# LargeWorldModel/LWM

Hardware: NVIDIA H100
Metric: ring_attn_fwd_bwd_tokens_per_s_attention_only_7B_128K (higher is better)
Workload: dtype bf16

## Files before the change

lwm_b200/csrc/attn_fwd.cu:

```cuda
#include "attn_common.cuh"
#include "tmap.h"
#include "capi_internal.h"

namespace lwm {

struct FwdParams {
  int B, H, Sq, Sk;
  float scale_log2;
  MaskParams mask;
  __nv_bfloat16* out;
  float* out_f32;
  float* lse;
  float* acc_o;
  float* acc_m;
  float* acc_l;
  int first, last;
  const float *scale_q, *scale_k, *scale_v;
};

constexpr int kFwdStages = 4;
constexpr int kFwdTileBytes = kTile * kHeadDim * 2;
constexpr int kFwdThreads = 384;
constexpr int kFwdConsumerWarps = 8;
constexpr int kFwdSmemBytes = (1 + kFwdStages) * kFwdTileBytes + 1024;

struct FwdBarriers {
  uint64_t q_full;
  uint64_t kv_full[kFwdStages];
  uint64_t kv_empty[kFwdStages];
};

LWM_DEVICE void load_tile(uint8_t* dst, const CUtensorMap* tm, uint64_t* bar, int h, int row0, int b) {
  mbar_arrive_expect_tx(bar, kFwdTileBytes);
  tma_load_4d(dst, tm, bar, 0, h, row0, b);
  tma_load_4d(dst + kFwdTileBytes / 2, tm, bar, 64, h, row0, b);
}

LWM_DEVICE float quad_max(float x) {
  x = fmaxf(x, __shfl_xor_sync(0xffffffffu, x, 1));
  return fmaxf(x, __shfl_xor_sync(0xffffffffu, x, 2));
}
LWM_DEVICE float quad_sum(float x) {
  x += __shfl_xor_sync(0xffffffffu, x, 1);
  return x + __shfl_xor_sync(0xffffffffu, x, 2);
}

template <bool kF16>
__global__ void __launch_bounds__(kFwdThreads, 1)
attn_fwd_kernel(const __grid_constant__ CUtensorMap tmQ, const __grid_constant__ CUtensorMap tmK,
                const __grid_constant__ CUtensorMap tmV, const FwdParams p) {
  extern __shared__ uint8_t smem_raw[];
  uint8_t* smem = reinterpret_cast<uint8_t*>((reinterpret_cast<uintptr_t>(smem_raw) + 1023) & ~uintptr_t(1023));
  uint8_t* sQ = smem;
  uint8_t* sKV = smem + kFwdTileBytes;
  __shared__ FwdBarriers bars;

  const int warp = threadIdx.x >> 5;
  const int lane = threadIdx.x & 31;
  const int n_q_tiles = p.Sq / kTile;
  const int tile = n_q_tiles - 1 - int(blockIdx.x);
  const int h = blockIdx.y, b = blockIdx.z;
  const int m0 = tile * kTile;

  int n_kv = p.Sk / kTile;
  if (p.mask.causal) {
    const long long last_q = (long long)p.mask.q_pos0 + m0 + kTile - 1;
    const long long vis = last_q - p.mask.k_pos0;
    n_kv = vis < 0 ? 0 : min((long long)n_kv, vis / kTile + 1);
  }
  if (n_kv == 0 && !p.first && !p.last) return;

  if (threadIdx.x == 0) {
    mbar_init(&bars.q_full, 1);
    for (int i = 0; i < kFwdStages; ++i) {
      mbar_init(&bars.kv_full[i], 1);
      mbar_init(&bars.kv_empty[i], kFwdConsumerWarps);
    }
    fence_mbar_init();
  }
  __syncthreads();

  if (warp >= 8) {
    setmaxnreg_dec<40>();
    if (warp == 8 && lane == 0 && n_kv > 0) {
      tma_prefetch_desc(&tmQ);
      tma_prefetch_desc(&tmK);
      tma_prefetch_desc(&tmV);
      load_tile(sQ, &tmQ, &bars.q_full, h, m0, b);
      for (int i = 0; i < 2 * n_kv; ++i) {
        const int slot = i % kFwdStages;
        const uint32_t ph = (i / kFwdStages) & 1;
        mbar_wait(&bars.kv_empty[slot], ph ^ 1);
        load_tile(sKV + slot * kFwdTileBytes, (i & 1) ? &tmV : &tmK, &bars.kv_full[slot], h, (i >> 1) * kTile, b);
      }
    }
    return;
  }

  setmaxnreg_inc<232>();
  const int wg = warp >> 2;
  const int w = warp & 3;
  const int quad = lane & 3;
  const int r0 = m0 + wg * 64 + w * 16 + (lane >> 2);
  const float scale = p.scale_log2 * (p.scale_q ? (*p.scale_q) * (*p.scale_k) : 1.0f);
  const bool has_bias = p.mask.bias != nullptr, has_seg = p.mask.seg != nullptr;
  const float* bias_row = has_bias ? p.mask.bias + (long long)b * p.mask.bias_stride : nullptr;
  const int* seg_row = has_seg ? p.mask.seg + (long long)b * p.mask.seg_stride : nullptr;
  long long q_pos[2];
  int my_seg[2];
#pragma unroll
  for (int hh = 0; hh < 2; ++hh) {
    q_pos[hh] = (long long)p.mask.q_pos0 + r0 + 8 * hh;
    my_seg[hh] = has_seg ? seg_row[q_pos[hh]] : 0;
  }

  float o[64];
#pragma unroll
  for (int i = 0; i < 64; ++i) o[i] = 0.f;
  float m_run[2] = {-INFINITY, -INFINITY}, l_run[2] = {0.f, 0.f};

  if (n_kv > 0) {
    mbar_wait(&bars.q_full, 0);
    const uint64_t q_desc = desc_kmajor_sw128(smem_u32(sQ + wg * 64 * 128));
    const uint32_t kv_base = smem_u32(sKV);
    const long long warp_q_pos0 = (long long)p.mask.q_pos0 + m0 + wg * 64 + w * 16;
    for (int j = 0; j < n_kv; ++j) {
      const int ik = 2 * j, iv = 2 * j + 1;
      float s[64];
      mbar_wait(&bars.kv_full[ik % kFwdStages], (ik / kFwdStages) & 1);
      const uint64_t kd = desc_kmajor_sw128(kv_base + (ik % kFwdStages) * kFwdTileBytes);
      wgmma_fence();
#pragma unroll
      for (int ks = 0; ks < kHeadDim / 16; ++ks) {
        const uint32_t off = (ks >> 2) * (kFwdTileBytes / 2) + (ks & 3) * 32;
        wgmma_ss<128, kF16, 0, 0>(s, desc_advance(q_desc, off), desc_advance(kd, off), ks > 0);
      }
      wgmma_commit();
      wgmma_wait<0>();
      reg_fence(s);
      if (lane == 0) mbar_arrive(&bars.kv_empty[ik % kFwdStages]);

      const long long k_tile_pos = (long long)p.mask.k_pos0 + (long long)j * kTile;
      const bool need_mask = has_bias || has_seg || (p.mask.causal && (k_tile_pos + kTile - 1 > warp_q_pos0));
      float mx[2] = {-INFINITY, -INFINITY};
      if (!need_mask) {
#pragma unroll
        for (int i = 0; i < 64; ++i) mx[(i >> 1) & 1] = fmaxf(mx[(i >> 1) & 1], s[i]);
        mx[0] = quad_max(mx[0]) * scale;
        mx[1] = quad_max(mx[1]) * scale;
      } else {
#pragma unroll
        for (int i = 0; i < 64; ++i) {
          const int hh = (i >> 1) & 1;
          const int col = (i >> 2) * 8 + quad * 2 + (i & 1);
          float tv = s[i] * scale;
          if (has_bias) {
            const float bt = bias_row[k_tile_pos + col] * kLog2e;
            tv = (bt < kMaskedLogit) ? kMaskedLogit : tv + bt;
          }
          if (has_seg && seg_row[k_tile_pos + col] != my_seg[hh]) tv = kMaskedLogit;
          if (p.mask.causal && k_tile_pos + col > q_pos[hh]) tv = kMaskedLogit;
          s[i] = tv;
          mx[hh] = fmaxf(mx[hh], tv);
        }
        mx[0] = quad_max(mx[0]);
        mx[1] = quad_max(mx[1]);
      }
      float alpha[2];
#pragma unroll
      for (int hh = 0; hh < 2; ++hh) {
        const float m_new = fmaxf(m_run[hh], mx[hh]);
        alpha[hh] = (m_run[hh] == -INFINITY) ? 0.f : ex2f(m_run[hh] - m_new);
        m_run[hh] = m_new;
        l_run[hh] *= alpha[hh];
      }
      if (j > 0) {
#pragma unroll
        for (int i = 0; i < 64; ++i) o[i] *= alpha[(i >> 1) & 1];
      }
      const float neg_m[2] = {-m_run[0], -m_run[1]};
      uint32_t pa[8][4];
#pragma unroll
      for (int kk = 0; kk < 8; ++kk) {
        float e[8];
#pragma unroll
        for (int t = 0; t < 8; ++t) {
          const int i = 8 * kk + t;
          const int hh = (t >> 1) & 1;
          e[t] = need_mask ? ex2f(s[i] + neg_m[hh]) : ex2f(fmaf(s[i], scale, neg_m[hh]));
          l_run[hh] += e[t];
        }
#pragma unroll
        for (int t = 0; t < 4; ++t) pa[kk][t] = kF16 ? pack_f16x2(e[2 * t], e[2 * t + 1]) : pack_bf16x2(e[2 * t], e[2 * t + 1]);
      }

      mbar_wait(&bars.kv_full[iv % kFwdStages], (iv / kFwdStages) & 1);
      const uint64_t vd = desc_mnmajor_sw128(kv_base + (iv % kFwdStages) * kFwdTileBytes, kFwdTileBytes / 2);
      reg_fence(o);
      wgmma_fence();
#pragma unroll
      for (int kk = 0; kk < kTile / 16; ++kk) wgmma_rs128<kF16, 1>(o, pa[kk], desc_advance(vd, kk * 2048), 1);
      wgmma_commit();
      wgmma_wait<0>();
      reg_fence(o);
      if (lane == 0) mbar_arrive(&bars.kv_empty[iv % kFwdStages]);
    }
  }

#pragma unroll
  for (int hh = 0; hh < 2; ++hh) {
    const int q_row = r0 + 8 * hh;
    const float l_run_row = quad_sum(l_run[hh]);
    const long long ml_idx = ((long long)b * p.H + h) * p.Sq + q_row;
    const long long o_idx = (((long long)b * p.Sq + q_row) * p.H + h) * kHeadDim;
    float m_c = -INFINITY, l_c = 0.f;
    if (!p.first) {
      m_c = p.acc_m[ml_idx];
      l_c = p.acc_l[ml_idx];
    }
    const float m_new = fmaxf(m_c, m_run[hh]);
    float wa = (m_c == -INFINITY) ? 0.f : ex2f(m_c - m_new);
    float wb = (m_run[hh] == -INFINITY) ? 0.f : ex2f(m_run[hh] - m_new);
    const float l_new = wa * l_c + wb * l_run_row;
    if (p.scale_v) wb *= *p.scale_v;
    if (p.last) {
      const float inv = l_new > 0.f ? 1.0f / l_new : 0.f;
      wa *= inv;
      wb *= inv;
    }
#pragma unroll
    for (int g = 0; g < kHeadDim / 8; ++g) {
      const int c = g * 8 + quad * 2;
      float2 f = make_float2(o[4 * g + 2 * hh] * wb, o[4 * g + 2 * hh + 1] * wb);
      if (!p.first) {
        const float2 a2 = *reinterpret_cast<const float2*>(p.acc_o + o_idx + c);
        f.x = fmaf(a2.x, wa, f.x);
        f.y = fmaf(a2.y, wa, f.y);
      }
      if (p.last) {
        *reinterpret_cast<uint32_t*>(p.out + o_idx + c) = pack_bf16x2(f.x, f.y);
        if (p.out_f32) *reinterpret_cast<float2*>(p.out_f32 + o_idx + c) = f;
      } else {
        *reinterpret_cast<float2*>(p.acc_o + o_idx + c) = f;
      }
    }
    if (quad == 0) {
      if (p.last) {
        p.lse[ml_idx] = l_new > 0.f ? (m_new + log2f(l_new)) * kLn2 : -INFINITY;
      } else {
        p.acc_m[ml_idx] = m_new;
        p.acc_l[ml_idx] = l_new;
      }
    }
  }
}

static bool make_qkv_tmap(CUtensorMap* tm, const void* ptr, int B, int S, int H) {
  uint64_t dims[4] = {uint64_t(kHeadDim), uint64_t(H), uint64_t(S), uint64_t(B)};
  uint64_t strides[3] = {uint64_t(kHeadDim) * 2, uint64_t(H) * kHeadDim * 2, uint64_t(S) * H * kHeadDim * 2};
  uint32_t box[4] = {64, 1, uint32_t(kTile), 1};
  return encode_tmap(tm, CU_TENSOR_MAP_DATA_TYPE_BFLOAT16, 4, ptr, dims, strides, box, CU_TENSOR_MAP_SWIZZLE_128B);
}

}

using namespace lwm;

static int attn_fwd_launch(const void* q, const void* k, const void* v, void* out, float* lse, float* acc_o,
                           float* acc_m, float* acc_l, int B, int H, int Sq, int Sk, int D, long long q_pos0,
                           long long k_pos0, int causal, const float* bias, long long bias_stride,
                           const int* segment_ids, long long seg_stride, float softmax_scale, int first, int last,
                           const float* scale_q, const float* scale_k, const float* scale_v, float* out_f32,
                           void* stream) {
  if (D != kHeadDim) return lwm_fail(LWM_ERR_SHAPE, "attn_fwd: head_dim must be 128");
  if (B <= 0 || H <= 0 || Sq <= 0 || Sk <= 0 || Sq % kTile || Sk % kTile)
    return lwm_fail(LWM_ERR_SHAPE, "attn_fwd: Sq and Sk must be positive multiples of 128");
  if (!q || !k || !v) return lwm_fail(LWM_ERR_ARG, "attn_fwd: null q/k/v");
  if (last && (!out || !lse)) return lwm_fail(LWM_ERR_ARG, "attn_fwd: out/lse required on the last step");
  if (!(first && last) && (!acc_o || !acc_m || !acc_l))
    return lwm_fail(LWM_ERR_ARG, "attn_fwd: carry buffers required unless first && last");
  if (q_pos0 + Sq > 0x7fffffffLL || k_pos0 + Sk > 0x7fffffffLL)
    return lwm_fail(LWM_ERR_SHAPE, "attn_fwd: global positions must fit in int32");
  if (bias && bias_stride < k_pos0 + Sk)
    return lwm_fail(LWM_ERR_SHAPE, "attn_fwd: bias is indexed by GLOBAL key position: bias_stride < k_pos0 + Sk");
  if (segment_ids && (seg_stride < q_pos0 + Sq || seg_stride < k_pos0 + Sk))
    return lwm_fail(LWM_ERR_SHAPE, "attn_fwd: segment_ids is indexed by GLOBAL position: seg_stride < max(q_pos0 + Sq, k_pos0 + Sk)");
  if (!lwm_check_device()) return LWM_ERR_DEVICE;
  CUtensorMap tq, tk, tv;
  if (!make_qkv_tmap(&tq, q, B, Sq, H) || !make_qkv_tmap(&tk, k, B, Sk, H) || !make_qkv_tmap(&tv, v, B, Sk, H))
    return lwm_fail(LWM_ERR_CUDA, "attn_fwd: cuTensorMapEncodeTiled failed (pointers must be 16B aligned)");
  FwdParams p;
  p.B = B; p.H = H; p.Sq = Sq; p.Sk = Sk;
  p.scale_log2 = softmax_scale * kLog2e;
  p.mask.q_pos0 = int(q_pos0); p.mask.k_pos0 = int(k_pos0); p.mask.causal = causal;
  p.mask.bias = bias; p.mask.bias_stride = bias_stride;
  p.mask.seg = segment_ids; p.mask.seg_stride = seg_stride;
  p.out = reinterpret_cast<__nv_bfloat16*>(out);
  p.lse = lse; p.acc_o = acc_o; p.acc_m = acc_m; p.acc_l = acc_l;
  p.first = first; p.last = last;
  p.scale_q = scale_q; p.scale_k = scale_k; p.scale_v = scale_v;
  p.out_f32 = out_f32;
  static bool attr_set_dev[64] = {};
  int cur_dev = 0;
  cudaGetDevice(&cur_dev);
  bool& attr_set = attr_set_dev[cur_dev & 63];
  if (!attr_set) {
    if (cudaFuncSetAttribute(attn_fwd_kernel<false>, cudaFuncAttributeMaxDynamicSharedMemorySize, kFwdSmemBytes) !=
            cudaSuccess ||
        cudaFuncSetAttribute(attn_fwd_kernel<true>, cudaFuncAttributeMaxDynamicSharedMemorySize, kFwdSmemBytes) !=
            cudaSuccess)
      return lwm_fail(LWM_ERR_CUDA, "attn_fwd: cannot raise dynamic shared memory limit");
    attr_set = true;
  }
  dim3 grid(Sq / kTile, H, B);
  if (scale_q)
    attn_fwd_kernel<true><<<grid, kFwdThreads, kFwdSmemBytes, reinterpret_cast<cudaStream_t>(stream)>>>(tq, tk, tv, p);
  else
    attn_fwd_kernel<false><<<grid, kFwdThreads, kFwdSmemBytes, reinterpret_cast<cudaStream_t>(stream)>>>(tq, tk, tv, p);
  return lwm_check_launch("attn_fwd_kernel");
}

extern "C" int lwm_attn_fwd_step(const void* q, const void* k, const void* v, void* out, float* lse, float* acc_o,
                                 float* acc_m, float* acc_l, int B, int H, int Sq, int Sk, int D,
                                 long long q_pos0, long long k_pos0, int causal, const float* bias,
                                 long long bias_stride, const int* segment_ids, long long seg_stride,
                                 float softmax_scale, int first, int last, void* stream) {
  return attn_fwd_launch(q, k, v, out, lse, acc_o, acc_m, acc_l, B, H, Sq, Sk, D, q_pos0, k_pos0, causal, bias,
                         bias_stride, segment_ids, seg_stride, softmax_scale, first, last, nullptr, nullptr, nullptr, nullptr, stream);
}

extern "C" int lwm_attn_fwd_step_f16(const void* q16, const void* k16, const void* v16, const float* scale_q,
                                     const float* scale_k, const float* scale_v, float* out_f32,
                                     void* out, float* lse, float* acc_o, float* acc_m, float* acc_l, int B, int H,
                                     int Sq, int Sk, int D, long long q_pos0, long long k_pos0, int causal,
                                     const float* bias, long long bias_stride, const int* segment_ids,
                                     long long seg_stride, float softmax_scale, int first, int last, void* stream) {
  if (!scale_q || !scale_k || !scale_v) return lwm_fail(LWM_ERR_ARG, "attn_fwd_f16: scales required");
  return attn_fwd_launch(q16, k16, v16, out, lse, acc_o, acc_m, acc_l, B, H, Sq, Sk, D, q_pos0, k_pos0, causal, bias,
                         bias_stride, segment_ids, seg_stride, softmax_scale, first, last, scale_q, scale_k, scale_v,
                         out_f32, stream);
}
```

lwm_b200/csrc/ptx.cuh:

```cuda
#pragma once
#include <cuda.h>
#include <cuda_runtime.h>
#include <cuda_bf16.h>
#include <stdint.h>
#include "wgmma.cuh"

namespace lwm {

#define LWM_DEVICE __device__ __forceinline__

LWM_DEVICE uint32_t smem_u32(const void* p) {
  return static_cast<uint32_t>(__cvta_generic_to_shared(p));
}
LWM_DEVICE uint32_t lane_id() { return threadIdx.x & 31; }

LWM_DEVICE void mbar_init(uint64_t* bar, uint32_t count) {
  asm volatile("mbarrier.init.shared::cta.b64 [%0], %1;" ::"r"(smem_u32(bar)), "r"(count) : "memory");
}
LWM_DEVICE void fence_mbar_init() { asm volatile("fence.mbarrier_init.release.cluster;" ::: "memory"); }
LWM_DEVICE void fence_proxy_async_smem() { asm volatile("fence.proxy.async.shared::cta;" ::: "memory"); }

LWM_DEVICE void mbar_arrive_expect_tx(uint64_t* bar, uint32_t bytes) {
  asm volatile("mbarrier.arrive.expect_tx.shared::cta.b64 _, [%0], %1;" ::"r"(smem_u32(bar)), "r"(bytes)
               : "memory");
}
LWM_DEVICE void mbar_arrive(uint64_t* bar) {
  asm volatile("mbarrier.arrive.shared::cta.b64 _, [%0];" ::"r"(smem_u32(bar)) : "memory");
}
LWM_DEVICE bool mbar_try_wait(uint64_t* bar, uint32_t parity) {
  uint32_t ok;
  asm volatile(
      "{\n\t.reg .pred P;\n\t"
      "mbarrier.try_wait.parity.shared::cta.b64 P, [%1], %2;\n\t"
      "selp.b32 %0, 1, 0, P;\n\t}\n"
      : "=r"(ok)
      : "r"(smem_u32(bar)), "r"(parity)
      : "memory");
  return ok != 0;
}
LWM_DEVICE void mbar_wait(uint64_t* bar, uint32_t parity) {
  while (!mbar_try_wait(bar, parity)) {
  }
}

LWM_DEVICE void tma_prefetch_desc(const CUtensorMap* m) {
  asm volatile("prefetch.tensormap [%0];" ::"l"(reinterpret_cast<uint64_t>(m)) : "memory");
}
LWM_DEVICE void tma_load_2d(void* smem_dst, const CUtensorMap* m, uint64_t* bar, int c0, int c1) {
  asm volatile(
      "cp.async.bulk.tensor.2d.shared::cluster.global.mbarrier::complete_tx::bytes [%0], [%1, {%3, %4}], [%2];"
      ::"r"(smem_u32(smem_dst)), "l"(reinterpret_cast<uint64_t>(m)), "r"(smem_u32(bar)), "r"(c0), "r"(c1)
      : "memory");
}
LWM_DEVICE void tma_load_3d(void* smem_dst, const CUtensorMap* m, uint64_t* bar, int c0, int c1, int c2) {
  asm volatile(
      "cp.async.bulk.tensor.3d.shared::cluster.global.mbarrier::complete_tx::bytes [%0], [%1, {%3, %4, %5}], [%2];"
      ::"r"(smem_u32(smem_dst)), "l"(reinterpret_cast<uint64_t>(m)), "r"(smem_u32(bar)), "r"(c0), "r"(c1), "r"(c2)
      : "memory");
}
LWM_DEVICE void tma_load_4d(void* smem_dst, const CUtensorMap* m, uint64_t* bar, int c0, int c1, int c2,
                            int c3) {
  asm volatile(
      "cp.async.bulk.tensor.4d.shared::cluster.global.mbarrier::complete_tx::bytes [%0], [%1, {%3, %4, %5, %6}], "
      "[%2];" ::"r"(smem_u32(smem_dst)),
      "l"(reinterpret_cast<uint64_t>(m)), "r"(smem_u32(bar)), "r"(c0), "r"(c1), "r"(c2), "r"(c3)
      : "memory");
}
LWM_DEVICE void bulk_load_1d(void* smem_dst, const void* gsrc, uint32_t bytes, uint64_t* bar) {
  asm volatile("cp.async.bulk.shared::cluster.global.mbarrier::complete_tx::bytes [%0], [%1], %2, [%3];" ::"r"(
                   smem_u32(smem_dst)),
               "l"(reinterpret_cast<uint64_t>(gsrc)), "r"(bytes), "r"(smem_u32(bar))
               : "memory");
}
LWM_DEVICE void tma_store_4d(const CUtensorMap* m, const void* smem_src, int c0, int c1, int c2, int c3) {
  asm volatile(
      "cp.async.bulk.tensor.4d.global.shared::cta.bulk_group [%0, {%2, %3, %4, %5}], [%1];" ::"l"(
          reinterpret_cast<uint64_t>(m)),
      "r"(smem_u32(smem_src)), "r"(c0), "r"(c1), "r"(c2), "r"(c3)
      : "memory");
}
LWM_DEVICE void tma_reduce_add_4d(const CUtensorMap* m, const void* smem_src, int c0, int c1, int c2, int c3) {
  asm volatile(
      "cp.reduce.async.bulk.tensor.4d.global.shared::cta.add.tile.bulk_group [%0, {%2, %3, %4, %5}], [%1];" ::"l"(
          reinterpret_cast<uint64_t>(m)),
      "r"(smem_u32(smem_src)), "r"(c0), "r"(c1), "r"(c2), "r"(c3)
      : "memory");
}
LWM_DEVICE void tma_commit_group() { asm volatile("cp.async.bulk.commit_group;" ::: "memory"); }
template <int N>
LWM_DEVICE void tma_wait_group_read() {
  asm volatile("cp.async.bulk.wait_group.read %0;" ::"n"(N) : "memory");
}
template <int N>
LWM_DEVICE void tma_wait_group() {
  asm volatile("cp.async.bulk.wait_group %0;" ::"n"(N) : "memory");
}

constexpr uint64_t kSwz128 = 1;
LWM_DEVICE uint64_t make_smem_desc(uint32_t saddr, uint32_t lbo_bytes, uint32_t sbo_bytes) {
  uint64_t d = 0;
  d |= static_cast<uint64_t>((saddr & 0x3FFFF) >> 4);
  d |= static_cast<uint64_t>((lbo_bytes >> 4) & 0x3FFF) << 16;
  d |= static_cast<uint64_t>((sbo_bytes >> 4) & 0x3FFF) << 32;
  d |= kSwz128 << 62;
  return d;
}
LWM_DEVICE uint64_t desc_kmajor_sw128(uint32_t saddr) { return make_smem_desc(saddr, 16, 1024); }
LWM_DEVICE uint64_t desc_mnmajor_sw128(uint32_t saddr, uint32_t mn_chunk_stride) {
  return make_smem_desc(saddr, mn_chunk_stride, 1024);
}

LWM_DEVICE uint64_t desc_advance(uint64_t d, uint32_t bytes) {
  const uint32_t lo = static_cast<uint32_t>(d) + (bytes >> 4);
  return (d & 0xFFFFFFFF00000000ull) | lo;
}

LWM_DEVICE void wgmma_fence() { asm volatile("wgmma.fence.sync.aligned;" ::: "memory"); }
LWM_DEVICE void wgmma_commit() { asm volatile("wgmma.commit_group.sync.aligned;" ::: "memory"); }
template <int N>
LWM_DEVICE void wgmma_wait() {
  asm volatile("wgmma.wait_group.sync.aligned %0;" ::"n"(N) : "memory");
}
template <int N>
LWM_DEVICE void reg_fence(float (&r)[N]) {
#pragma unroll
  for (int i = 0; i < N; ++i) asm volatile("" : "+f"(r[i])::"memory");
}
template <int N>
LWM_DEVICE void reg_fence(uint32_t (&r)[N]) {
#pragma unroll
  for (int i = 0; i < N; ++i) asm volatile("" : "+r"(r[i])::"memory");
}

LWM_DEVICE uint32_t pack_bf16x2(float lo, float hi) {
  uint32_t r;
  asm("cvt.rn.bf16x2.f32 %0, %1, %2;" : "=r"(r) : "f"(hi), "f"(lo));
  return r;
}
LWM_DEVICE uint32_t pack_f16x2(float lo, float hi) {
  uint32_t r;
  asm("cvt.rn.f16x2.f32 %0, %1, %2;" : "=r"(r) : "f"(hi), "f"(lo));
  return r;
}
LWM_DEVICE float ex2f(float x) {
  float y;
  asm("ex2.approx.ftz.f32 %0, %1;" : "=f"(y) : "f"(x));
  return y;
}
template <int kRegs>
LWM_DEVICE void setmaxnreg_inc() {
  asm volatile("setmaxnreg.inc.sync.aligned.u32 %0;" ::"n"(kRegs));
}
template <int kRegs>
LWM_DEVICE void setmaxnreg_dec() {
  asm volatile("setmaxnreg.dec.sync.aligned.u32 %0;" ::"n"(kRegs));
}
LWM_DEVICE void named_bar_sync(uint32_t id, uint32_t nthreads) {
  asm volatile("bar.sync %0, %1;" ::"r"(id), "r"(nthreads) : "memory");
}

LWM_DEVICE uint32_t swz128_offset(uint32_t row, uint32_t chunk16) {
  return row * 128u + ((chunk16 ^ (row & 7u)) << 4);
}

}
```

Measured before the change: 4093.

## Software-pipeline QK^T and PV wgmmas with ping-pong warpgroup scheduling in forward

Restructures the forward consumer loop so the S=QK^T wgmma for tile j is issued together with the PV wgmma for tile j-1. The softmax of tile j then overlaps the in-flight PV matmul. Named barriers alternate the two consumer warpgroups (ping-pong) so one issues tensor-core work while the other does softmax. Register budgets shift from 40/232 to 24/240 to hold the extra live state (s, pa, o). Mask setup moves inside the masked branch and position math is narrowed to int, which risks overflow for very long positions.

Measured after the change: 4227 (median of 6 runs). 1.03x the previous value.

```diff
diff --git a/lwm_b200/csrc/attn_fwd.cu b/lwm_b200/csrc/attn_fwd.cu
--- a/lwm_b200/csrc/attn_fwd.cu
+++ b/lwm_b200/csrc/attn_fwd.cu
@@ -81,7 +81,7 @@
   __syncthreads();
 
   if (warp >= 8) {
-    setmaxnreg_dec<40>();
+    setmaxnreg_dec<24>();
     if (warp == 8 && lane == 0 && n_kv > 0) {
       tma_prefetch_desc(&tmQ);
       tma_prefetch_desc(&tmK);
@@ -97,22 +97,13 @@
     return;
   }
 
-  setmaxnreg_inc<232>();
+  setmaxnreg_inc<240>();
   const int wg = warp >> 2;
   const int w = warp & 3;
   const int quad = lane & 3;
   const int r0 = m0 + wg * 64 + w * 16 + (lane >> 2);
   const float scale = p.scale_log2 * (p.scale_q ? (*p.scale_q) * (*p.scale_k) : 1.0f);
   const bool has_bias = p.mask.bias != nullptr, has_seg = p.mask.seg != nullptr;
-  const float* bias_row = has_bias ? p.mask.bias + (long long)b * p.mask.bias_stride : nullptr;
-  const int* seg_row = has_seg ? p.mask.seg + (long long)b * p.mask.seg_stride : nullptr;
-  long long q_pos[2];
-  int my_seg[2];
-#pragma unroll
-  for (int hh = 0; hh < 2; ++hh) {
-    q_pos[hh] = (long long)p.mask.q_pos0 + r0 + 8 * hh;
-    my_seg[hh] = has_seg ? seg_row[q_pos[hh]] : 0;
-  }
 
   float o[64];
 #pragma unroll
@@ -123,24 +114,37 @@
     mbar_wait(&bars.q_full, 0);
     const uint64_t q_desc = desc_kmajor_sw128(smem_u32(sQ + wg * 64 * 128));
     const uint32_t kv_base = smem_u32(sKV);
-    const long long warp_q_pos0 = (long long)p.mask.q_pos0 + m0 + wg * 64 + w * 16;
-    for (int j = 0; j < n_kv; ++j) {
-      const int ik = 2 * j, iv = 2 * j + 1;
-      float s[64];
-      mbar_wait(&bars.kv_full[ik % kFwdStages], (ik / kFwdStages) & 1);
-      const uint64_t kd = desc_kmajor_sw128(kv_base + (ik % kFwdStages) * kFwdTileBytes);
-      wgmma_fence();
+    const int warp_q_pos0 = p.mask.q_pos0 + m0 + wg * 64 + w * 16;
+    float s[64];
+    uint32_t pa[8][4];
+    float alpha[2];
+
+    auto wait_full = [&](int i) { mbar_wait(&bars.kv_full[i % kFwdStages], (i / kFwdStages) & 1); };
+    auto release = [&](int i) {
+      if (lane == 0) mbar_arrive(&bars.kv_empty[i % kFwdStages]);
+    };
+    auto turn_begin = [&]() { named_bar_sync(1 + wg, 256); };
+    auto turn_end = [&](bool last) {
+      if (!(last && wg == 1)) named_bar_arrive(2 - wg, 256);
+    };
+    if (wg == 1) named_bar_arrive(1, 256);
+    auto issue_s = [&](int j) {
+      const uint64_t kd = desc_kmajor_sw128(kv_base + ((2 * j) % kFwdStages) * kFwdTileBytes);
 #pragma unroll
       for (int ks = 0; ks < kHeadDim / 16; ++ks) {
         const uint32_t off = (ks >> 2) * (kFwdTileBytes / 2) + (ks & 3) * 32;
         wgmma_ss<128, kF16, 0, 0>(s, desc_advance(q_desc, off), desc_advance(kd, off), ks > 0);
       }
       wgmma_commit();
-      wgmma_wait<0>();
-      reg_fence(s);
-      if (lane == 0) mbar_arrive(&bars.kv_empty[ik % kFwdStages]);
-
-      const long long k_tile_pos = (long long)p.mask.k_pos0 + (long long)j * kTile;
+    };
+    auto issue_pv = [&](int j) {
+      const uint64_t vd = desc_mnmajor_sw128(kv_base + ((2 * j + 1) % kFwdStages) * kFwdTileBytes, kFwdTileBytes / 2);
+#pragma unroll
+      for (int kk = 0; kk < kTile / 16; ++kk) wgmma_rs128<kF16, 1>(o, pa[kk], desc_advance(vd, kk * 2048), 1);
+      wgmma_commit();
+    };
+    auto softmax = [&](int j) {
+      const int k_tile_pos = p.mask.k_pos0 + j * kTile;
       const bool need_mask = has_bias || has_seg || (p.mask.causal && (k_tile_pos + kTile - 1 > warp_q_pos0));
       float mx[2] = {-INFINITY, -INFINITY};
       if (!need_mask) {
@@ -149,6 +153,15 @@
         mx[0] = quad_max(mx[0]) * scale;
         mx[1] = quad_max(mx[1]) * scale;
       } else {
+        const float* bias_row = has_bias ? p.mask.bias + (long long)b * p.mask.bias_stride : nullptr;
+        const int* seg_row = has_seg ? p.mask.seg + (long long)b * p.mask.seg_stride : nullptr;
+        int q_pos[2];
+        int my_seg[2];
+#pragma unroll
+        for (int hh = 0; hh < 2; ++hh) {
+          q_pos[hh] = p.mask.q_pos0 + r0 + 8 * hh;
+          my_seg[hh] = has_seg ? seg_row[q_pos[hh]] : 0;
+        }
 #pragma unroll
         for (int i = 0; i < 64; ++i) {
           const int hh = (i >> 1) & 1;
@@ -166,45 +179,70 @@
         mx[0] = quad_max(mx[0]);
         mx[1] = quad_max(mx[1]);
       }
-      float alpha[2];
 #pragma unroll
       for (int hh = 0; hh < 2; ++hh) {
         const float m_new = fmaxf(m_run[hh], mx[hh]);
         alpha[hh] = (m_run[hh] == -INFINITY) ? 0.f : ex2f(m_run[hh] - m_new);
         m_run[hh] = m_new;
-        l_run[hh] *= alpha[hh];
-      }
-      if (j > 0) {
-#pragma unroll
-        for (int i = 0; i < 64; ++i) o[i] *= alpha[(i >> 1) & 1];
+        l_run[hh] = __fmul_rn(l_run[hh], alpha[hh]);
       }
       const float neg_m[2] = {-m_run[0], -m_run[1]};
-      uint32_t pa[8][4];
-#pragma unroll
-      for (int kk = 0; kk < 8; ++kk) {
-        float e[8];
-#pragma unroll
-        for (int t = 0; t < 8; ++t) {
-          const int i = 8 * kk + t;
-          const int hh = (t >> 1) & 1;
-          e[t] = need_mask ? ex2f(s[i] + neg_m[hh]) : ex2f(fmaf(s[i], scale, neg_m[hh]));
-          l_run[hh] += e[t];
+#pragma unroll
+      for (int i = 0; i < 64; ++i) {
+        const int hh = (i >> 1) & 1;
+        s[i] = need_mask ? ex2f(s[i] + neg_m[hh]) : ex2f(fmaf(s[i], scale, neg_m[hh]));
+        l_run[hh] += s[i];
+      }
+    };
+    auto pack_p = [&]() {
+#pragma unroll
+      for (int kk = 0; kk < 8; ++kk)
+#pragma unroll
+        for (int t = 0; t < 4; ++t) {
+          const int i = 8 * kk + 2 * t;
+          pa[kk][t] = kF16 ? pack_f16x2(s[i], s[i + 1]) : pack_bf16x2(s[i], s[i + 1]);
         }
-#pragma unroll
-        for (int t = 0; t < 4; ++t) pa[kk][t] = kF16 ? pack_f16x2(e[2 * t], e[2 * t + 1]) : pack_bf16x2(e[2 * t], e[2 * t + 1]);
-      }
-
-      mbar_wait(&bars.kv_full[iv % kFwdStages], (iv / kFwdStages) & 1);
-      const uint64_t vd = desc_mnmajor_sw128(kv_base + (iv % kFwdStages) * kFwdTileBytes, kFwdTileBytes / 2);
+    };
+
+    wait_full(0);
+    turn_begin();
+    wgmma_fence();
+    issue_s(0);
+    turn_end(false);
+    wgmma_wait<0>();
+    reg_fence(s);
+    release(0);
+    softmax(0);
+    pack_p();
+    for (int j = 1; j < n_kv; ++j) {
+      wait_full(2 * j);
+      wait_full(2 * j - 1);
+      turn_begin();
       reg_fence(o);
       wgmma_fence();
-#pragma unroll
-      for (int kk = 0; kk < kTile / 16; ++kk) wgmma_rs128<kF16, 1>(o, pa[kk], desc_advance(vd, kk * 2048), 1);
-      wgmma_commit();
+      issue_s(j);
+      issue_pv(j - 1);
+      turn_end(false);
+      wgmma_wait<1>();
+      reg_fence(s);
+      release(2 * j);
+      softmax(j);
       wgmma_wait<0>();
       reg_fence(o);
-      if (lane == 0) mbar_arrive(&bars.kv_empty[iv % kFwdStages]);
-    }
+      release(2 * j - 1);
+#pragma unroll
+      for (int i = 0; i < 64; ++i) o[i] *= alpha[(i >> 1) & 1];
+      pack_p();
+    }
+    wait_full(2 * n_kv - 1);
+    turn_begin();
+    reg_fence(o);
+    wgmma_fence();
+    issue_pv(n_kv - 1);
+    turn_end(true);
+    wgmma_wait<0>();
+    reg_fence(o);
+    release(2 * n_kv - 1);
   }
 
 #pragma unroll
diff --git a/lwm_b200/csrc/ptx.cuh b/lwm_b200/csrc/ptx.cuh
--- a/lwm_b200/csrc/ptx.cuh
+++ b/lwm_b200/csrc/ptx.cuh
@@ -158,6 +158,9 @@
 LWM_DEVICE void named_bar_sync(uint32_t id, uint32_t nthreads) {
   asm volatile("bar.sync %0, %1;" ::"r"(id), "r"(nthreads) : "memory");
 }
+LWM_DEVICE void named_bar_arrive(uint32_t id, uint32_t nthreads) {
+  asm volatile("bar.arrive %0, %1;" ::"r"(id), "r"(nthreads) : "memory");
+}
 
 LWM_DEVICE uint32_t swz128_offset(uint32_t row, uint32_t chunk16) {
   return row * 128u + ((chunk16 ^ (row & 7u)) << 4);
```
